# Visual-Behavior/aloception-oss

Measured on AMD Instinct MI355X. Metric: frames/sec (whole node) DeformableDETR-R50 inference, higher is better.
Workload: dtype bf16; 1 GPU; DeformableDETR-R50 inference bf16, batch 8 synthetic 1333x800 frames per GPU, random-init weights; launch=hip-graph replay + eager inference(), per_gpu_batch=8, global_batch=8, parallelism=batch-sharded x1, no collective

## Files before the change

### aloception-oss_amd/csrc/stem.hip

```cpp
#include "common.hpp"

namespace alo {
namespace {

constexpr int kPoolRows = 8, kPoolCols = 7;
constexpr int kConvRows = 2 * kPoolRows + 1, kConvCols = 2 * kPoolCols + 1;
constexpr int kConvPix = kConvRows * kConvCols;
constexpr int kInRows = 2 * kConvRows + 5 + 1;
constexpr int kInCols = 2 * kConvCols + 5;
constexpr int kInElems = kInCols * 3;
constexpr int kInStride = 224;
constexpr int kConvStride = 64 * 2 + 16;
constexpr int kKsteps = 11;
constexpr int kStemThreads = 256;
constexpr int kStemLds = kInRows * kInStride + kConvPix * kConvStride + 64 * 4;
static_assert(kConvPix <= 8 * 32, "8 MFMA row tiles");

struct StemDims {
    int N, H, W, Hc, Wc, Hp, Wp;
    long sN, sC, sH, sW;
    int tiles_y, tiles_x;
};

__device__ __forceinline__ unsigned max_u16x2(unsigned a, unsigned b) {
    typedef unsigned short u16x2 __attribute__((ext_vector_type(2)));
    union { unsigned u; u16x2 v; } x, y, z;
    x.u = a; y.u = b;
    z.v = __builtin_elementwise_max(x.v, y.v);
    return z.u;
}

__global__ void __launch_bounds__(kStemThreads, 2)
stem_conv_pool_kernel(const bf16_t* __restrict__ X, const bf16_t* __restrict__ Wp, const bf16_t* __restrict__ bias,
                      bf16_t* __restrict__ Y, const StemDims dm) {
    extern __shared__ __attribute__((aligned(16))) unsigned char smem[];
    unsigned char* const in_lds = smem;
    unsigned char* const conv_lds = smem + kInRows * kInStride;
    const int tid = threadIdx.x, wave = tid >> 6, lane = tid & 63, nl = lane & 31, kg = lane >> 5;

    u32x4 wreg[kKsteps][2];
#pragma unroll
    for (int s = 0; s < kKsteps; ++s)
#pragma unroll
        for (int ct = 0; ct < 2; ++ct) wreg[s][ct] = *reinterpret_cast<const u32x4*>(Wp + ((size_t)(ct * kKsteps + s) * 64 + lane) * 8);
    float* const bias_lds = reinterpret_cast<float*>(smem + kInRows * kInStride + kConvPix * kConvStride);
    if (tid < 64) {
        const int r = tid & 15, ct = (tid >> 4) & 1, k2 = tid >> 5;
        bias_lds[tid] = bias ? bf16_to_f32(bias[32 * ct + (r & 3) + 8 * (r >> 2) + 4 * k2].bits) : 0.f;
    }

    for (int i = tid; i < kInRows * (kInStride / 2 - kInElems); i += kStemThreads) {
        const int row = i / (kInStride / 2 - kInElems), e = kInElems + i % (kInStride / 2 - kInElems);
        *reinterpret_cast<uint16_t*>(in_lds + row * kInStride + e * 2) = 0;
    }

    const int tiles_per_image = dm.tiles_y * dm.tiles_x;
    const int ntiles = tiles_per_image * dm.N;

    constexpr int kStageIters = (kInRows * kInElems + kStemThreads - 1) / kStemThreads;
    uint16_t sv[kStageIters];
    auto load_tile = [&](int tl) {
        const int n = tl / tiles_per_image, trem = tl - n * tiles_per_image;
        const int ty = trem / dm.tiles_x, tx = trem - ty * dm.tiles_x;
        const int iy0 = 4 * ty * kPoolRows - 5, ix0 = 4 * tx * kPoolCols - 5;
        const bf16_t* xn = X + (size_t)n * dm.sN;
#pragma unroll
        for (int it = 0; it < kStageIters; ++it) {
            const int i = tid + it * kStemThreads;
            const int row = i / kInElems, e = i - row * kInElems, xc = e / 3, c = e - 3 * xc;
            const int iy = iy0 + row, ix = ix0 + xc;
            const bool ok = i < kInRows * kInElems && iy >= 0 && iy < dm.H && ix >= 0 && ix < dm.W;
            sv[it] = ok ? xn[c * dm.sC + iy * dm.sH + ix * dm.sW].bits : (uint16_t)0;
        }
    };
    if ((int)blockIdx.x < ntiles) load_tile(blockIdx.x);

    for (int tile = blockIdx.x; tile < ntiles; tile += gridDim.x) {
        const int n = tile / tiles_per_image, trem = tile - n * tiles_per_image;
        const int ty = trem / dm.tiles_x, tx = trem - ty * dm.tiles_x;
        const int py0 = ty * kPoolRows, px0 = tx * kPoolCols;
        const int cy0 = 2 * py0 - 1, cx0 = 2 * px0 - 1;

#pragma unroll
        for (int it = 0; it < kStageIters; ++it) {
            const int i = tid + it * kStemThreads;
            const int row = i / kInElems, e = i - row * kInElems;
            if (i < kInRows * kInElems) *reinterpret_cast<uint16_t*>(in_lds + row * kInStride + e * 2) = sv[it];
        }
        __syncthreads();
        if (tile + (int)gridDim.x < ntiles) load_tile(tile + gridDim.x);

#pragma unroll 1
        for (int half = 0; half < 2; ++half) {
            const int rt = wave + 4 * half;
            const int m_raw = rt * 32 + nl;
            const int m = m_raw < kConvPix ? m_raw : kConvPix - 1;
            const int lr = m / kConvCols, lc = m - lr * kConvCols;
            const unsigned char* a_base = in_lds + (2 * lr) * kInStride + lc * 12;
            f32x16 acc[2];
#pragma unroll
            for (int ct = 0; ct < 2; ++ct)
#pragma unroll
                for (int q = 0; q < 4; ++q) {
                    const f32x4 b4 = *reinterpret_cast<const f32x4*>(bias_lds + (kg * 2 + ct) * 16 + 4 * q);
#pragma unroll
                    for (int i = 0; i < 4; ++i) acc[ct][4 * q + i] = b4[i];
                }
#pragma unroll
            for (int s = 0; s < kKsteps; ++s) {
                const int g0 = 2 * s, g1 = 2 * s + 1;
                const int off = kg ? (g1 / 3) * kInStride + (g1 % 3) * 16 : (g0 / 3) * kInStride + (g0 % 3) * 16;
                const unsigned* ap = reinterpret_cast<const unsigned*>(a_base + off);
                u32x4 a = {ap[0], ap[1], ap[2], ap[3]};
                const int G = kg ? g1 : g0;
                if (G == 21) a = u32x4{0u, 0u, 0u, 0u};
                else if (G % 3 == 2) { a.z &= 0x0000ffffu; a.w = 0u; }
#pragma unroll
                for (int ct = 0; ct < 2; ++ct)
                    acc[ct] = mfma_32x32x16<bf16_t>(wreg[s][ct], a, acc[ct]);
            }
            const int cy = cy0 + lr, cx = cx0 + lc;
            const bool ok = cy >= 0 && cy < dm.Hc && cx >= 0 && cx < dm.Wc;
            if (m_raw < kConvPix) {
#pragma unroll
                for (int ct = 0; ct < 2; ++ct)
#pragma unroll
                    for (int q = 0; q < 4; ++q) {
                        unsigned lo = 0u, hi = 0u;
                        if (ok) {
                            const float v0 = acc[ct][4 * q], v1 = acc[ct][4 * q + 1], v2 = acc[ct][4 * q + 2], v3 = acc[ct][4 * q + 3];
                            lo = pack_bf16x2(relu_keep_nan(v0), relu_keep_nan(v1));
                            hi = pack_bf16x2(relu_keep_nan(v2), relu_keep_nan(v3));
                        }
                        *reinterpret_cast<u32x2*>(conv_lds + m * kConvStride + (32 * ct + 8 * q + 4 * kg) * 2) = u32x2{lo, hi};
                    }
            }
        }
        __syncthreads();

        if (tid < kPoolRows * kPoolCols * 4) {
            const int pp = tid >> 2, cg = tid & 3;
            const int lpy = pp / kPoolCols, lpx = pp - lpy * kPoolCols;
            u32x4 m0 = {0u, 0u, 0u, 0u}, m1 = {0u, 0u, 0u, 0u};
#pragma unroll
            for (int dy = 0; dy < 3; ++dy)
#pragma unroll
                for (int dx = 0; dx < 3; ++dx) {
                    const unsigned char* p = conv_lds + ((2 * lpy + dy) * kConvCols + 2 * lpx + dx) * kConvStride + cg * 32;
                    const u32x4 v0 = *reinterpret_cast<const u32x4*>(p), v1 = *reinterpret_cast<const u32x4*>(p + 16);
#pragma unroll
                    for (int j = 0; j < 4; ++j) {
                        m0[j] = max_u16x2(m0[j], v0[j]);
                        m1[j] = max_u16x2(m1[j], v1[j]);
                    }
                }
            const int py = py0 + lpy, px = px0 + lpx;
            if (py < dm.Hp && px < dm.Wp) {
                bf16_t* o = Y + (((size_t)n * dm.Hp + py) * dm.Wp + px) * 64 + cg * 16;
                *reinterpret_cast<u32x4*>(o) = m0;
                *reinterpret_cast<u32x4*>(o + 8) = m1;
            }
        }
        __syncthreads();
    }
}

}
}

using namespace alo;

extern "C" int alo_stem_conv_pool(const void* x, const void* w_packed, const void* bias, void* y, int N, int H, int W,
                                  long stride_n, long stride_c, long stride_h, long stride_w, int dtype, void* stream) {
    ALO_REQUIRE(x && w_packed && y, ALO_ERR_INVALID_ARGUMENT, "alo_stem_conv_pool: null pointer argument");
    ALO_REQUIRE(N > 0 && H > 0 && W > 0, ALO_ERR_INVALID_ARGUMENT, "alo_stem_conv_pool: N, H, W must be positive");
    ALO_REQUIRE(dtype == ALO_BF16, ALO_ERR_UNSUPPORTED, "alo_stem_conv_pool: bf16 only (dtype %d)", dtype);
    ALO_REQUIRE(aligned16(w_packed, y), ALO_ERR_INVALID_ARGUMENT, "alo_stem_conv_pool: w_packed and y must be 16-byte aligned");
    StemDims dm;
    dm.N = N; dm.H = H; dm.W = W;
    dm.Hc = (H - 1) / 2 + 1; dm.Wc = (W - 1) / 2 + 1;
    dm.Hp = (dm.Hc - 1) / 2 + 1; dm.Wp = (dm.Wc - 1) / 2 + 1;
    dm.sN = stride_n; dm.sC = stride_c; dm.sH = stride_h; dm.sW = stride_w;
    dm.tiles_y = (dm.Hp + kPoolRows - 1) / kPoolRows;
    dm.tiles_x = (dm.Wp + kPoolCols - 1) / kPoolCols;
    const long ntiles = (long)dm.tiles_y * dm.tiles_x * N;
    ALO_REQUIRE(ntiles < (1L << 30), ALO_ERR_UNSUPPORTED, "alo_stem_conv_pool: image batch too large");
    void* args[] = {&x, &w_packed, &bias, &y, &dm};
    const unsigned grid = (unsigned)(ntiles < 768 ? ntiles : 768);
    return launch<stem_conv_pool_kernel>(grid, kStemThreads, kStemLds, static_cast<hipStream_t>(stream), "alo_stem_conv_pool", args);
}
```

Before: 936.3 frames/s.

## Add row-vectorized stem staging kernel with deeper prefetch and CU-sized grid

Adds a new stem conv+pool kernel that stages input rows with one aligned dword load per thread, specialised for planar or interleaved input layouts, replacing the scalar per-element gather. It prefetches two tiles ahead, parking the next tile into LDS during pooling. It also raises residency to 3 blocks per CU and sizes the grid from the CU count instead of a fixed 768. The stem is a small part of the full DeformableDETR forward, and the higher occupancy target may add register pressure.

```diff
diff --git a/aloception-oss_amd/csrc/stem.hip b/aloception-oss_amd/csrc/stem.hip
--- a/aloception-oss_amd/csrc/stem.hip
+++ b/aloception-oss_amd/csrc/stem.hip
@@ -1,3 +1,6 @@
+#include <cstdlib>
+#include <cstring>
+
 #include "common.hpp"
 
 namespace alo {
@@ -13,6 +16,7 @@
 constexpr int kConvStride = 64 * 2 + 16;
 constexpr int kKsteps = 11;
 constexpr int kStemThreads = 256;
+constexpr int kStemResident = 3;
 constexpr int kStemLds = kInRows * kInStride + kConvPix * kConvStride + 64 * 4;
 static_assert(kConvPix <= 8 * 32, "8 MFMA row tiles");
 
@@ -28,6 +32,102 @@
     x.u = a; y.u = b;
     z.v = __builtin_elementwise_max(x.v, y.v);
     return z.u;
+}
+
+__device__ __forceinline__ void conv_tile(const unsigned char* in_lds, unsigned char* conv_lds, const float* bias_lds,
+                                          const u32x4 (&wreg)[kKsteps][2], int cy0, int cx0, const StemDims& dm, int wave, int nl, int kg) {
+#pragma unroll 1
+    for (int half = 0; half < 2; ++half) {
+        const int rt = wave + 4 * half;
+        const int m_raw = rt * 32 + nl;
+        const int m = m_raw < kConvPix ? m_raw : kConvPix - 1;
+        const int lr = m / kConvCols, lc = m - lr * kConvCols;
+        const unsigned char* a_base = in_lds + (2 * lr) * kInStride + lc * 12;
+        f32x16 acc[2];
+#pragma unroll
+        for (int ct = 0; ct < 2; ++ct)
+#pragma unroll
+            for (int q = 0; q < 4; ++q) {
+                const f32x4 b4 = *reinterpret_cast<const f32x4*>(bias_lds + (kg * 2 + ct) * 16 + 4 * q);
+#pragma unroll
+                for (int i = 0; i < 4; ++i) acc[ct][4 * q + i] = b4[i];
+            }
+#pragma unroll
+        for (int s = 0; s < kKsteps; ++s) {
+            const int g0 = 2 * s, g1 = 2 * s + 1;
+            const int off = kg ? (g1 / 3) * kInStride + (g1 % 3) * 16 : (g0 / 3) * kInStride + (g0 % 3) * 16;
+            const unsigned* ap = reinterpret_cast<const unsigned*>(a_base + off);
+            u32x4 a = {ap[0], ap[1], ap[2], ap[3]};
+            const int G = kg ? g1 : g0;
+            if (G == 21) a = u32x4{0u, 0u, 0u, 0u};
+            else if (G % 3 == 2) { a.z &= 0x0000ffffu; a.w = 0u; }
+#pragma unroll
+            for (int ct = 0; ct < 2; ++ct)
+                acc[ct] = mfma_32x32x16<bf16_t>(wreg[s][ct], a, acc[ct]);
+        }
+        const int cy = cy0 + lr, cx = cx0 + lc;
+        const bool ok = cy >= 0 && cy < dm.Hc && cx >= 0 && cx < dm.Wc;
+        if (m_raw < kConvPix) {
+#pragma unroll
+            for (int ct = 0; ct < 2; ++ct)
+#pragma unroll
+                for (int q = 0; q < 4; ++q) {
+                    unsigned lo = 0u, hi = 0u;
+                    if (ok) {
+                        const float v0 = acc[ct][4 * q], v1 = acc[ct][4 * q + 1], v2 = acc[ct][4 * q + 2], v3 = acc[ct][4 * q + 3];
+                        lo = pack_bf16x2(relu_keep_nan(v0), relu_keep_nan(v1));
+                        hi = pack_bf16x2(relu_keep_nan(v2), relu_keep_nan(v3));
+                    }
+                    *reinterpret_cast<u32x2*>(conv_lds + m * kConvStride + (32 * ct + 8 * q + 4 * kg) * 2) = u32x2{lo, hi};
+                }
+        }
+    }
+}
+
+__device__ __forceinline__ void pool_tile(const unsigned char* conv_lds, bf16_t* __restrict__ Y, int n, int py0, int px0,
+                                          const StemDims& dm, int tid) {
+    if (tid < kPoolRows * kPoolCols * 4) {
+        const int pp = tid >> 2, cg = tid & 3;
+        const int lpy = pp / kPoolCols, lpx = pp - lpy * kPoolCols;
+        u32x4 m0 = {0u, 0u, 0u, 0u}, m1 = {0u, 0u, 0u, 0u};
+#pragma unroll
+        for (int dy = 0; dy < 3; ++dy)
+#pragma unroll
+            for (int dx = 0; dx < 3; ++dx) {
+                const unsigned char* p = conv_lds + ((2 * lpy + dy) * kConvCols + 2 * lpx + dx) * kConvStride + cg * 32;
+                const u32x4 v0 = *reinterpret_cast<const u32x4*>(p), v1 = *reinterpret_cast<const u32x4*>(p + 16);
+#pragma unroll
+                for (int j = 0; j < 4; ++j) {
+                    m0[j] = max_u16x2(m0[j], v0[j]);
+                    m1[j] = max_u16x2(m1[j], v1[j]);
+                }
+            }
+        const int py = py0 + lpy, px = px0 + lpx;
+        if (py < dm.Hp && px < dm.Wp) {
+            bf16_t* o = Y + (((size_t)n * dm.Hp + py) * dm.Wp + px) * 64 + cg * 16;
+            *reinterpret_cast<u32x4*>(o) = m0;
+            *reinterpret_cast<u32x4*>(o + 8) = m1;
+        }
+    }
+}
+
+__device__ __forceinline__ void stem_setup(const bf16_t* __restrict__ Wp, const bf16_t* __restrict__ bias, unsigned char* smem,
+                                           u32x4 (&wreg)[kKsteps][2], int tid, int lane) {
+    unsigned char* const in_lds = smem;
+#pragma unroll
+    for (int s = 0; s < kKsteps; ++s)
+#pragma unroll
+        for (int ct = 0; ct < 2; ++ct) wreg[s][ct] = *reinterpret_cast<const u32x4*>(Wp + ((size_t)(ct * kKsteps + s) * 64 + lane) * 8);
+    float* const bias_lds = reinterpret_cast<float*>(smem + kInRows * kInStride + kConvPix * kConvStride);
+    if (tid < 64) {
+        const int r = tid & 15, ct = (tid >> 4) & 1, k2 = tid >> 5;
+        bias_lds[tid] = bias ? bf16_to_f32(bias[32 * ct + (r & 3) + 8 * (r >> 2) + 4 * k2].bits) : 0.f;
+    }
+
+    for (int i = tid; i < kInRows * (kInStride / 2 - kInElems); i += kStemThreads) {
+        const int row = i / (kInStride / 2 - kInElems), e = kInElems + i % (kInStride / 2 - kInElems);
+        *reinterpret_cast<uint16_t*>(in_lds + row * kInStride + e * 2) = 0;
+    }
 }
 
 __global__ void __launch_bounds__(kStemThreads, 2)
@@ -38,21 +138,9 @@
     unsigned char* const conv_lds = smem + kInRows * kInStride;
     const int tid = threadIdx.x, wave = tid >> 6, lane = tid & 63, nl = lane & 31, kg = lane >> 5;
 
+    float* const bias_lds = reinterpret_cast<float*>(smem + kInRows * kInStride + kConvPix * kConvStride);
     u32x4 wreg[kKsteps][2];
-#pragma unroll
-    for (int s = 0; s < kKsteps; ++s)
-#pragma unroll
-        for (int ct = 0; ct < 2; ++ct) wreg[s][ct] = *reinterpret_cast<const u32x4*>(Wp + ((size_t)(ct * kKsteps + s) * 64 + lane) * 8);
-    float* const bias_lds = reinterpret_cast<float*>(smem + kInRows * kInStride + kConvPix * kConvStride);
-    if (tid < 64) {
-        const int r = tid & 15, ct = (tid >> 4) & 1, k2 = tid >> 5;
-        bias_lds[tid] = bias ? bf16_to_f32(bias[32 * ct + (r & 3) + 8 * (r >> 2) + 4 * k2].bits) : 0.f;
-    }
-
-    for (int i = tid; i < kInRows * (kInStride / 2 - kInElems); i += kStemThreads) {
-        const int row = i / (kInStride / 2 - kInElems), e = kInElems + i % (kInStride / 2 - kInElems);
-        *reinterpret_cast<uint16_t*>(in_lds + row * kInStride + e * 2) = 0;
-    }
+    stem_setup(Wp, bias, smem, wreg, tid, lane);
 
     const int tiles_per_image = dm.tiles_y * dm.tiles_x;
     const int ntiles = tiles_per_image * dm.N;
@@ -90,77 +178,95 @@
         __syncthreads();
         if (tile + (int)gridDim.x < ntiles) load_tile(tile + gridDim.x);
 
-#pragma unroll 1
-        for (int half = 0; half < 2; ++half) {
-            const int rt = wave + 4 * half;
-            const int m_raw = rt * 32 + nl;
-            const int m = m_raw < kConvPix ? m_raw : kConvPix - 1;
-            const int lr = m / kConvCols, lc = m - lr * kConvCols;
-            const unsigned char* a_base = in_lds + (2 * lr) * kInStride + lc * 12;
-            f32x16 acc[2];
-#pragma unroll
-            for (int ct = 0; ct < 2; ++ct)
-#pragma unroll
-                for (int q = 0; q < 4; ++q) {
-                    const f32x4 b4 = *reinterpret_cast<const f32x4*>(bias_lds + (kg * 2 + ct) * 16 + 4 * q);
-#pragma unroll
-                    for (int i = 0; i < 4; ++i) acc[ct][4 * q + i] = b4[i];
-                }
-#pragma unroll
-            for (int s = 0; s < kKsteps; ++s) {
-                const int g0 = 2 * s, g1 = 2 * s + 1;
-                const int off = kg ? (g1 / 3) * kInStride + (g1 % 3) * 16 : (g0 / 3) * kInStride + (g0 % 3) * 16;
-                const unsigned* ap = reinterpret_cast<const unsigned*>(a_base + off);
-                u32x4 a = {ap[0], ap[1], ap[2], ap[3]};
-                const int G = kg ? g1 : g0;
-                if (G == 21) a = u32x4{0u, 0u, 0u, 0u};
-                else if (G % 3 == 2) { a.z &= 0x0000ffffu; a.w = 0u; }
-#pragma unroll
-                for (int ct = 0; ct < 2; ++ct)
-                    acc[ct] = mfma_32x32x16<bf16_t>(wreg[s][ct], a, acc[ct]);
-            }
-            const int cy = cy0 + lr, cx = cx0 + lc;
-            const bool ok = cy >= 0 && cy < dm.Hc && cx >= 0 && cx < dm.Wc;
-            if (m_raw < kConvPix) {
-#pragma unroll
-                for (int ct = 0; ct < 2; ++ct)
-#pragma unroll
-                    for (int q = 0; q < 4; ++q) {
-                        unsigned lo = 0u, hi = 0u;
-                        if (ok) {
-                            const float v0 = acc[ct][4 * q], v1 = acc[ct][4 * q + 1], v2 = acc[ct][4 * q + 2], v3 = acc[ct][4 * q + 3];
-                            lo = pack_bf16x2(relu_keep_nan(v0), relu_keep_nan(v1));
-                            hi = pack_bf16x2(relu_keep_nan(v2), relu_keep_nan(v3));
-                        }
-                        *reinterpret_cast<u32x2*>(conv_lds + m * kConvStride + (32 * ct + 8 * q + 4 * kg) * 2) = u32x2{lo, hi};
-                    }
-            }
-        }
-        __syncthreads();
-
-        if (tid < kPoolRows * kPoolCols * 4) {
-            const int pp = tid >> 2, cg = tid & 3;
-            const int lpy = pp / kPoolCols, lpx = pp - lpy * kPoolCols;
-            u32x4 m0 = {0u, 0u, 0u, 0u}, m1 = {0u, 0u, 0u, 0u};
-#pragma unroll
-            for (int dy = 0; dy < 3; ++dy)
-#pragma unroll
-                for (int dx = 0; dx < 3; ++dx) {
-                    const unsigned char* p = conv_lds + ((2 * lpy + dy) * kConvCols + 2 * lpx + dx) * kConvStride + cg * 32;
-                    const u32x4 v0 = *reinterpret_cast<const u32x4*>(p), v1 = *reinterpret_cast<const u32x4*>(p + 16);
-#pragma unroll
-                    for (int j = 0; j < 4; ++j) {
-                        m0[j] = max_u16x2(m0[j], v0[j]);
-                        m1[j] = max_u16x2(m1[j], v1[j]);
-                    }
-                }
-            const int py = py0 + lpy, px = px0 + lpx;
-            if (py < dm.Hp && px < dm.Wp) {
-                bf16_t* o = Y + (((size_t)n * dm.Hp + py) * dm.Wp + px) * 64 + cg * 16;
-                *reinterpret_cast<u32x4*>(o) = m0;
-                *reinterpret_cast<u32x4*>(o + 8) = m1;
-            }
-        }
+        conv_tile(in_lds, conv_lds, bias_lds, wreg, cy0, cx0, dm, wave, nl, kg);
+        __syncthreads();
+
+        pool_tile(conv_lds, Y, n, py0, px0, dm, tid);
+        __syncthreads();
+    }
+}
+
+enum StemLayout { kPlanar, kInterleaved };
+
+template <StemLayout LAYOUT>
+__global__ void __launch_bounds__(kStemThreads, kStemResident)
+stem_conv_pool_rows_kernel(const bf16_t* __restrict__ X, const bf16_t* __restrict__ Wp, const bf16_t* __restrict__ bias,
+                           bf16_t* __restrict__ Y, const StemDims dm) {
+    extern __shared__ __attribute__((aligned(16))) unsigned char smem[];
+    unsigned char* const in_lds = smem;
+    unsigned char* const conv_lds = smem + kInRows * kInStride;
+    const int tid = threadIdx.x, wave = tid >> 6, lane = tid & 63, nl = lane & 31, kg = lane >> 5;
+    float* const bias_lds = reinterpret_cast<float*>(smem + kInRows * kInStride + kConvPix * kConvStride);
+    u32x4 wreg[kKsteps][2];
+    stem_setup(Wp, bias, smem, wreg, tid, lane);
+
+    const int tiles_per_image = dm.tiles_y * dm.tiles_x;
+    const int ntiles = tiles_per_image * dm.N;
+
+    constexpr int kRunElems = LAYOUT == kPlanar ? kInCols : kInElems;
+    constexpr int kPerPixel = LAYOUT == kPlanar ? 1 : 3;
+    constexpr int kDwords = kRunElems / 2 + 1;
+    constexpr int kSlots = LAYOUT == kPlanar ? 12 : 4;
+    constexpr int kRowIters = kInRows / 4;
+    constexpr int kElemPitch = LAYOUT == kPlanar ? 6 : 2;
+    static_assert(kDwords * kSlots <= kStemThreads && kInRows % 4 == 0, "one dword per thread and row");
+    const int slot = tid / kDwords, j = tid - slot * kDwords;
+    const int c = LAYOUT == kPlanar ? slot % 3 : 0, rsub = LAYOUT == kPlanar ? slot / 3 : slot;
+    const bool stager = tid < kDwords * kSlots;
+
+    const long skew = (long)(reinterpret_cast<uintptr_t>(X) & 3);
+    const unsigned char* const xdw = reinterpret_cast<const unsigned char*>(X) - skew;
+    unsigned sv[kRowIters];
+    int sv_e = 0;
+    auto load_tile = [&](int tl) {
+        const int n = tl / tiles_per_image, trem = tl - n * tiles_per_image;
+        const int ty = trem / dm.tiles_x, tx = trem - ty * dm.tiles_x;
+        const int iy0 = 4 * ty * kPoolRows - 5, ix0 = 4 * tx * kPoolCols - 5;
+        const long image = skew + 2 * (long)n * dm.sN;
+        const long at = image + 2 * (c * dm.sC + (long)(iy0 + rsub) * dm.sH + (long)ix0 * kPerPixel + 2 * j);
+        const int e_lo = 2 * j - (int)((at >> 1) & 1);
+        const int first = ix0 < 0 ? -ix0 * kPerPixel : 0;
+        const int end = (dm.W - ix0) * kPerPixel < kRunElems ? (dm.W - ix0) * kPerPixel : kRunElems;
+        const unsigned keep = (e_lo >= first && e_lo < end ? 0x0000ffffu : 0u) | (e_lo + 1 >= first && e_lo + 1 < end ? 0xffff0000u : 0u);
+        const unsigned char* const p = xdw + (at & ~3L);
+        const unsigned char* const in_image = xdw + (image & ~3L);
+        sv_e = e_lo;
+#pragma unroll
+        for (int it = 0; it < kRowIters; ++it) {
+            const int iy = iy0 + rsub + 4 * it;
+            const bool ok = stager && keep != 0u && iy >= 0 && iy < dm.H;
+            const unsigned char* q = ok ? p + it * (8 * dm.sH) : in_image;
+            sv[it] = *reinterpret_cast<const unsigned*>(q) & (ok ? keep : 0u);
+        }
+    };
+    auto park_tile = [&]() {
+        unsigned char* const d = in_lds + rsub * kInStride + c * 2 + sv_e * kElemPitch;
+        if (stager && (unsigned)sv_e < (unsigned)kRunElems) {
+#pragma unroll
+            for (int it = 0; it < kRowIters; ++it) *reinterpret_cast<uint16_t*>(d + it * 4 * kInStride) = (uint16_t)sv[it];
+        }
+        if (stager && (unsigned)(sv_e + 1) < (unsigned)kRunElems) {
+#pragma unroll
+            for (int it = 0; it < kRowIters; ++it) *reinterpret_cast<uint16_t*>(d + kElemPitch + it * 4 * kInStride) = (uint16_t)(sv[it] >> 16);
+        }
+    };
+
+    const int step = gridDim.x;
+    int tile = blockIdx.x;
+    if (tile < ntiles) { load_tile(tile); park_tile(); }
+    if (tile + step < ntiles) load_tile(tile + step);
+    __syncthreads();
+    for (; tile < ntiles; tile += step) {
+        const int n = tile / tiles_per_image, trem = tile - n * tiles_per_image;
+        const int ty = trem / dm.tiles_x, tx = trem - ty * dm.tiles_x;
+        const int py0 = ty * kPoolRows, px0 = tx * kPoolCols;
+
+        conv_tile(in_lds, conv_lds, bias_lds, wreg, 2 * py0 - 1, 2 * px0 - 1, dm, wave, nl, kg);
+        __syncthreads();
+
+        if (tile + step < ntiles) park_tile();
+        if (tile + 2 * step < ntiles) load_tile(tile + 2 * step);
+        pool_tile(conv_lds, Y, n, py0, px0, dm, tid);
         __syncthreads();
     }
 }
@@ -186,6 +292,18 @@
     const long ntiles = (long)dm.tiles_y * dm.tiles_x * N;
     ALO_REQUIRE(ntiles < (1L << 30), ALO_ERR_UNSUPPORTED, "alo_stem_conv_pool: image batch too large");
     void* args[] = {&x, &w_packed, &bias, &y, &dm};
-    const unsigned grid = (unsigned)(ntiles < 768 ? ntiles : 768);
-    return launch<stem_conv_pool_kernel>(grid, kStemThreads, kStemLds, static_cast<hipStream_t>(stream), "alo_stem_conv_pool", args);
-}
+    hipStream_t s = static_cast<hipStream_t>(stream);
+    const char* knob = getenv("ALO_STEM");
+    const bool planar = stride_w == 1 && stride_h > 0 && stride_c >= 0 && stride_n >= 0;
+    const bool interleaved = stride_c == 1 && stride_w == 3 && stride_h > 0 && stride_n >= 0;
+    if ((knob && !strcmp(knob, "legacy")) || !(planar || interleaved)) {
+        const unsigned grid = (unsigned)(ntiles < 768 ? ntiles : 768);
+        return launch<stem_conv_pool_kernel>(grid, kStemThreads, kStemLds, s, "alo_stem_conv_pool", args);
+    }
+    int dev = 0, cus = 0;
+    if (hipGetDevice(&dev) != hipSuccess || hipDeviceGetAttribute(&cus, hipDeviceAttributeMultiprocessorCount, dev) != hipSuccess || cus < 1)
+        return fail(ALO_ERR_LAUNCH, "alo_stem_conv_pool: cannot read the device's compute unit count");
+    const unsigned grid = (unsigned)(ntiles < (long)kStemResident * cus ? ntiles : (long)kStemResident * cus);
+    return planar ? launch<stem_conv_pool_rows_kernel<kPlanar>>(grid, kStemThreads, kStemLds, s, "alo_stem_conv_pool", args)
+                  : launch<stem_conv_pool_rows_kernel<kInterleaved>>(grid, kStemThreads, kStemLds, s, "alo_stem_conv_pool", args);
+}
```

Result: no change. 945.1 frames/s (median of 6 runs) (+0.9%).
